# braingeneers/statdepth

Hardware: AMD Instinct MI355X
Metric: curve-pairs/sec (MBD) (higher is better)
Workload: dtype f64

## Files before the change

statdepth_amd/csrc/mbd_rank_bucket32.hip:

```cpp
#include <atomic>

#include "sd_common.h"
#include "rank_bucket.h"

namespace sd {

constexpr int R32_PRIO_LDS = 2;
constexpr int R32_PRIO_VALU = 0;
constexpr int R32_MIN_N = 3072;
constexpr int R32_LNB = 14;
constexpr int R32_NT = 512, R32_NW = 8;
constexpr int R32_LCAP = 64;
constexpr int R32_PAD = 12;
constexpr u32 R32_TB = 1024;
constexpr int R32_TSH = 30;
constexpr double R32_CDIV = 1.0 / 448.0;
constexpr double R32_BETA = 2.0;
constexpr u32 R32_SENT = 0x7FFFFFFFu;

template <int E, int LNB>
struct R32Cfg {
    static constexpr int NT = R32_NT, NW = R32_NW, NB = 1 << LNB;
    static constexpr int QW = NB / 2 / NT / 4;
    static_assert(QW >= 1 && NB / 2 == QW * 4 * NT, "whole quads of histogram words per thread");
    static constexpr int SH = 31 - LNB;
    static constexpr u32 C0 = R32_TB << SH, C1 = ((u32)NB - R32_TB) << SH;
    static constexpr u32 NANIMG = ((u32)NB + 2u) << SH;
    static_assert(LNB == 14, "the first tail octave continues the core's slope for 14 336 core buckets");
    static constexpr size_t HDR = 8 * NW * 8 + NW * 4 + 32 + (size_t)R32_LCAP * 8;
    static_assert(HDR % 16 == 0, "the histogram starts on a 16-byte boundary");
    static __host__ __device__ constexpr int al4(int n) { return (n + 3) & ~3; }
    static __host__ __device__ constexpr int pstride(int n) { return (n + 31) & ~31; }
    static __host__ __device__ constexpr int dummy_pos(int n) { return al4(n) + R32_PAD; }
    static __host__ __device__ constexpr size_t lds_bytes(int n) { return HDR + (size_t)(NB / 2 + 4) * 4 + (size_t)(dummy_pos(n) + 4) * 4; }
};

template <int E, int LNB>
__global__ __launch_bounds__(R32_NT, 4) void rank_bucket32_kernel(const double *__restrict__ Y, i64 n64, i64 row0, i64 rows,
                                                                 u32 *__restrict__ partial, unsigned char *__restrict__ rowflag,
                                                                 u32 *__restrict__ gate, u32 epoch, u64 *__restrict__ out_zero) {
    using C = R32Cfg<E, LNB>;
    constexpr int NT = C::NT, NW = C::NW, NB = C::NB, QW = C::QW, SH = C::SH;
    constexpr u32 C0 = C::C0, C1 = C::C1, NANIMG = C::NANIMG;
    extern __shared__ double Sm[];
    const int n = (int)n64;
    double *red = Sm;
    u32 *wtot = reinterpret_cast<u32 *>(red + 8 * NW);
    u32 *misc = wtot + NW;
    u32 *lkey = misc + 8, *lbe = lkey + R32_LCAP;
    u32 *H = reinterpret_cast<u32 *>(reinterpret_cast<char *>(Sm) + C::HDR);
    u32 *S = H + NB / 2 + 4;
    const unsigned short *H16 = reinterpret_cast<const unsigned short *>(H);
    const int t0 = threadIdx.x;
    const double INF = __builtin_huge_val();
    const double QNAN = __builtin_nan("");
    const int DUMMY = C::dummy_pos(n);
    const uint4 *SENT = reinterpret_cast<const uint4 *>(S + C::al4(n));
    const u32 nm1 = (u32)n - 1u;
    const u32 ranksum = (u32)(((u64)n * (u64)(n - 1)) >> 1);
    int t = t0;

    if (blockIdx.x == 0 && t == 0) gate[2] = 0;
    if (out_zero)
        for (i64 c = (i64)blockIdx.x * NT + t; c < n; c += (i64)gridDim.x * NT) out_zero[c] = 0;
    for (int p = n + t; p < DUMMY + 4; p += NT) S[p] = R32_SENT;
    {
        uint4 *Hq = reinterpret_cast<uint4 *>(H);
#pragma unroll
        for (int i = 0; i < QW; ++i) Hq[i * NT + t] = make_uint4(0, 0, 0, 0);
        if (t < 4) H[NB / 2 + t] = 0;
        if (t < 5) misc[t] = 0;
    }

    double x[E];
    auto load_row = [&](i64 r) {
        const double *rp = Y + (row0 + r) * n + t;
#pragma unroll
        for (int e = 0; e < E; ++e) x[e] = (e < E - 2 || t + e * NT < n) ? rp[e * NT] : QNAN;
    };
    u32 acc[E];
#pragma unroll
    for (int e = 0; e < E; ++e) acc[e] = 0;
    double smp;
    auto sample_issue = [&](i64 r) { smp = Y[(row0 + r) * n + (((((u32)t * 397u) & 511u) * (u32)n) >> 9)]; };
    auto row_range = [&](int parity) {
        double mn = INF, mx = -INF;
#pragma unroll
        for (int e = 0; e < E; ++e) {
            mn = rb_mm<false>(mn, x[e]);
            mx = rb_mm<true>(mx, x[e]);
        }
        mn = rb_wave_allreduce<false>(mn);
        mx = rb_wave_allreduce<true>(mx);
        const float sf = (float)smp;
        const float rmn = rb_row_allreduce_f32<false>(sf == sf ? sf : __builtin_huge_valf());
        const float rmx = rb_row_allreduce_f32<true>(sf == sf ? sf : -__builtin_huge_valf());
        auto rl = [](float v, int l) -> float { return __int_as_float(__builtin_amdgcn_readlane(__float_as_int(v), l)); };
        float imn = fmaxf(fmaxf(rl(rmn, 0), rl(rmn, 16)), fmaxf(rl(rmn, 32), rl(rmn, 48)));
        float imx = fminf(fminf(rl(rmx, 0), rl(rmx, 16)), fminf(rl(rmx, 32), rl(rmx, 48)));
        {
            bool eqs = false;
#define R32_NB(k) eqs = eqs || (__int_as_float(__builtin_amdgcn_mov_dpp(__float_as_int(sf), 0x120 + k, 0xF, 0xF, false)) == sf);
            R32_NB(1) R32_NB(2) R32_NB(3) R32_NB(4) R32_NB(5) R32_NB(6) R32_NB(7)
#undef R32_NB
            if (__ballot(eqs) != 0) { imn = __builtin_huge_valf(); imx = -__builtin_huge_valf(); }
        }
        double *rp = red + parity * 4 * NW;
        if ((t & 63) == 63) {
            double *wp = rp + 4 * (t >> 6);
            wp[0] = mn; wp[1] = mx;
            reinterpret_cast<float *>(wp + 2)[0] = imn;
            reinterpret_cast<float *>(wp + 2)[1] = imx;
        }
    };
    int par = 0;
    u32 rowidx = 0, nbad = 0, expect = 0;
    bool handover = false;
    bool stop = false;
    u32 kb[E];
    i64 r = blockIdx.x;
    for (; r < rows; r += gridDim.x) {
        t = t0;
        asm volatile("" : "+v"(t));
        const int lane = t & 63;
        const int wave = __builtin_amdgcn_readfirstlane(t >> 6);
        if (rowidx && t == 0) misc[3] = __hip_atomic_load(gate + 1, __ATOMIC_RELAXED, __HIP_MEMORY_SCOPE_AGENT);
        __builtin_amdgcn_s_setprio(R32_PRIO_LDS);
        sample_issue(r);
        load_row(r);
        row_range(par);
        double *redp = red + par * 4 * NW;
        par ^= 1;
        __syncthreads();
        if (rowidx) {
            const u32 w = misc[3];
            if ((w >> 8) == (epoch & 0xFFFFFFu) && (w & 0xFFu) >= 8u) { stop = true; break; }
        }
        double lo, hi;
        double mscale, moff, mc;
        u64 mcb;
        u32 mc0, mcw;
        bool go, bad;
        {
            const double2 p = reinterpret_cast<const double2 *>(redp)[2 * (lane & (NW - 1))];
            const float2 pb = reinterpret_cast<const float2 *>(redp + 4 * (lane & (NW - 1)) + 2)[0];
            lo = rb_readlane_f64(rb_row_allreduce<false>(p.x), 0);
            hi = rb_readlane_f64(rb_row_allreduce<true>(p.y), 0);
            const double imn = (double)__int_as_float(__builtin_amdgcn_readfirstlane(__float_as_int(rb_row_allreduce_f32<true>(pb.x))));
            const double imx = (double)__int_as_float(__builtin_amdgcn_readfirstlane(__float_as_int(rb_row_allreduce_f32<false>(pb.y))));
            const bool fin = (hi > lo) && (lo > -INF) && (hi < INF) && ((hi - lo) < INF);
            bad = !fin && (hi >= lo);
            const double si = imx - imn;
            u32 c0 = 256u, c1 = 0x7FFFFE00u;
            if (fin && si > 0.0 && si < INF && (hi - lo) > (1.5 * (1.0 + 2.0 * R32_BETA)) * si) {
                const double lo2 = imn - R32_BETA * si, hi2 = imx + R32_BETA * si;
                lo = lo2 > lo ? lo2 : lo;
                hi = hi2 < hi ? hi2 : hi;
                c0 = C0;
                c1 = C1;
            }
            mc0 = c0;
            mcw = c1 - c0;
            const double wc = hi - lo;
            mscale = ((double)mcw - 64.0) / wc;
            moff = __builtin_fma(-lo, mscale, (double)c0);
            mc = wc * R32_CDIV;
            mcb = (u64)__double_as_longlong(mc);
            go = fin && (wc > 0.0) && (mscale < INF) && (mc > 0.0);
            bad = bad || (fin && !go);
        }
        auto convert4 = [&](const double (&xv)[4], u32 (&q)[4]) {
            bool anyout = false;
#pragma unroll
            for (int i = 0; i < 4; ++i) {
                const double u = __builtin_fma(xv[i], mscale, moff);
                u32 qi;
                asm("v_cvt_u32_f64 %0, %1" : "=v"(qi) : "v"(u));
                q[i] = qi;
                anyout = anyout || (qi - mc0 >= mcw);
            }
            if (__ballot(anyout) != 0) {
#pragma unroll
                for (int i = 0; i < 4; ++i) {
                    const bool outc = q[i] - mc0 >= mcw, low = q[i] < mc0;
                    double d = low ? lo - xv[i] : xv[i] - hi;
                    d = rb_mm<true>(d, 0.0);
                    const u64 tc = ((u64)__double_as_longlong(d + mc) - mcb) >> R32_TSH;
                    const u32 room = low ? mc0 - 1u : 0x7FFFFEFFu - (mc0 + mcw);
                    const u32 tcc = tc < (u64)room ? (u32)tc : room;
                    u32 qt = low ? (mc0 - 1u) - tcc : (mc0 + mcw) + tcc;
                    qt = (xv[i] == xv[i]) ? qt : NANIMG;
                    q[i] = outc ? qt : q[i];
                }
            }
        };
        u32 sl[(E + 3) / 4];
        if (go) {
#pragma unroll
            for (int e = 0; e < (E + 3) / 4; ++e) sl[e] = 0;
#pragma unroll
            for (int e0 = 0; e0 < E; e0 += 8) {
                u32 old[8];
#pragma unroll
                for (int h = 0; h < 8; h += 4) {
                    if (e0 + h < E) {
                        double xv[4];
                        u32 q[4];
#pragma unroll
                        for (int i = 0; i < 4; ++i) xv[i] = e0 + h + i < E ? x[e0 + h + i] : x[e0 + h];
                        convert4(xv, q);
#pragma unroll
                        for (int i = 0; i < 4; ++i)
                            if (e0 + h + i < E) kb[e0 + h + i] = q[i];
                    }
                }
#pragma unroll
                for (int i = 0; i < 8; ++i) {
                    const int e = e0 + i;
                    if (e < E) {
                        const u32 b = kb[e] >> SH;
                        old[i] = atomicAdd(&H[b >> 1], 1u << ((b & 1u) * 16u));
                    }
                }
#pragma unroll
                for (int i = 0; i < 8; ++i) {
                    const int e = e0 + i;
                    if (e < E)
                        sl[e >> 2] |= ((old[i] >> (((kb[e] >> SH) & 1u) * 16u)) & 0xFFu) << (8 * (e & 3));
                }
                asm volatile("" : "+v"(sl[e0 >> 2]));
                if (e0 + 4 < E) asm volatile("" : "+v"(sl[(e0 >> 2) + 1]));
            }
            __syncthreads();
            uint4 *Hq = reinterpret_cast<uint4 *>(H) + wave * (64 * QW);
            uint4 hq[QW];
            u32 runq[QW], inclq[QW], offq[QW], ov = 0, wsum = 0;
#pragma unroll
            for (int i = 0; i < QW; ++i) {
                hq[i] = Hq[i * 64 + lane];
                const u32 s4 = hq[i].x + hq[i].y + hq[i].z + hq[i].w;
                ov |= hq[i].x | hq[i].y | hq[i].z | hq[i].w;
                runq[i] = (s4 & 0xFFFFu) + (s4 >> 16);
                inclq[i] = rb_wave_incl_scan(runq[i]);
                offq[i] = wsum;
                wsum += rb_readlane(inclq[i], 63);
            }
            const bool wover = __ballot((ov & 0xFFC0FFC0u) != 0) != 0;
            const bool wtry = __ballot((ov & 0xFFF0FFF0u) != 0) != 0;
            if (lane == 63) wtot[wave] = wsum | (wover ? 0x80000000u : 0u) | (wtry ? 0x40000000u : 0u);
            __syncthreads();
            const u32 wt = wtot[lane & (NW - 1)];
            const bool crowded = __ballot((wt >> 31) != 0) != 0;
            const bool trypure = __ballot((wt & 0x40000000u) != 0) != 0;
            const u32 wscan = rb_row_incl_scan(wt & 0x3FFFFFFFu);
            const u32 woff = wave ? rb_readlane(wscan, wave - 1) : 0u;
#pragma unroll
            for (int i = 0; i < QW; ++i) {
                u32 base = woff + offq[i] + inclq[i] - runq[i];
                uint4 o;
                o.x = base | ((base + (hq[i].x & 0xFFFFu)) << 16);
                base += (hq[i].x & 0xFFFFu) + (hq[i].x >> 16);
                o.y = base | ((base + (hq[i].y & 0xFFFFu)) << 16);
                base += (hq[i].y & 0xFFFFu) + (hq[i].y >> 16);
                o.z = base | ((base + (hq[i].z & 0xFFFFu)) << 16);
                base += (hq[i].z & 0xFFFFu) + (hq[i].z >> 16);
                o.w = base | ((base + (hq[i].w & 0xFFFFu)) << 16);
                base += (hq[i].w & 0xFFFFu) + (hq[i].w >> 16);
                Hq[i * 64 + lane] = o;
                if (i == QW - 1 && t == NT - 1) H[NB / 2] = base;
            }
            __syncthreads();
            const u32 nv = H[NB / 2];
            bool take = nv == (u32)n;
            u32 bc[E];
            if (take) {
#pragma unroll
                for (int e = 0; e < E; ++e) {
                    const u32 b = kb[e] >> SH, slot = (sl[e >> 2] >> (8 * (e & 3))) & 0xFFu;
                    u32 b1 = b + 1u;
                    asm("" : "+v"(b1));
                    const u32 base = H16[b], end = H16[b1];
                    const bool isk = e < E - 2 || t + e * NT < n;
                    S[isk ? base + slot : (u32)DUMMY] = kb[e];
                    bc[e] = isk ? base | ((end - base) << 14) : (1u << 14);
                }
            }
            __syncthreads();
            bool pure = false;
            if (take && (trypure || crowded)) {
                const u32 tag = rowidx + 1u;
                bool vote = false, same = true;
#pragma unroll
                for (int e = 0; e < E; ++e) {
                    const u32 base = bc[e] & 0x3FFFu, cnt = bc[e] >> 14;
                    if (e < E - 2 || t + e * NT < n) {
                        const u32 first = S[base];
                        same = same && (first == kb[e]);
                        if (cnt >= 16u) vote = vote || (first == kb[e] && S[base + 1] == kb[e]);
                    }
                }
                if (vote) misc[2] = tag;
                if (!same) misc[4] = tag;
                __syncthreads();
                if ((misc[2] == tag && misc[4] != tag) || crowded) {
                    take = false;
                    bool ok = misc[2] == tag && misc[4] != tag;
                    if (ok) {
                        const double *rp = Y + (row0 + r) * n + t;
#pragma unroll
                        for (int pass = 0; pass < 2; ++pass) {
                            bool eq = true;
#pragma unroll
                            for (int e0 = 0; e0 < E; e0 += 4) {
                                int eo = e0 * NT;
                                asm volatile("" : "+v"(eo));
                                const double *rq = rp + eo;
                                u64 w[4];
#pragma unroll
                                for (int i = 0; i < 4; ++i) {
                                    const bool isk = e0 + i < E && (e0 + i < E - 2 || t + (e0 + i) * NT < n);
                                    w[i] = (u64)__double_as_longlong((isk ? rq[i * NT] : 0.0) + 0.0);
                                }
#pragma unroll
                                for (int i = 0; i < 4; ++i) {
                                    if (e0 + i < E && (e0 + i < E - 2 || t + (e0 + i) * NT < n) && (bc[e0 + i] >> 14) >= 2u) {
                                        u32 *sp = S + (bc[e0 + i] & 0x3FFFu);
                                        if (pass == 0) { sp[0] = (u32)(w[i] >> 32); sp[1] = (u32)w[i]; }
                                        else eq = eq && sp[0] == (u32)(w[i] >> 32) && sp[1] == (u32)w[i];
                                    }
                                }
                                __builtin_amdgcn_sched_barrier(0);
                            }
                            if (pass == 1 && !eq) misc[4] = tag;
                            __syncthreads();
                        }
                        ok = misc[4] != tag;
                    }
                    if (ok) {
                        pure = true;
#pragma unroll
                        for (int e = 0; e < E; ++e) {
                            const u32 B = bc[e] & 0x3FFFu, A = (u32)n - B - (bc[e] >> 14);
                            acc[e] += (e < E - 2 || t + e * NT < n) ? (nm1 * (nm1 - 1u) - A * (A - 1u) - B * (B - 1u)) >> 1 : 0u;
                        }
                    }
                }
            }
            __builtin_amdgcn_s_setprio(R32_PRIO_VALU);
            {
                uint4 *Hz = reinterpret_cast<uint4 *>(H) + wave * (64 * QW);
#pragma unroll
                for (int i = 0; i < QW; ++i) Hz[i * 64 + lane] = make_uint4(0, 0, 0, 0);
                if (t < 2) H[NB / 2 + t] = 0;
            }
            if (take) {
                const uint4 *S4 = reinterpret_cast<const uint4 *>(S);
                uint4 y0, y1;
                auto window = [&](int e) {
                    const u32 base = bc[e] & 0x3FFFu, cnt = bc[e] >> 14;
                    const uint4 *p = S4 + (base >> 2);
                    y0 = p[0];
                    y1 = *((cnt + (base & 3u) > 4u) ? p + 1 : SENT);
                };
                u32 sB = 0;
                window(0);
#pragma unroll
                for (int e = 0; e < E; ++e) {
                    const u32 base = bc[e] & 0x3FFFu, cnt = bc[e] >> 14, off = base & 3u;
                    const u32 qe = kb[e];
                    u32 lt = 0;
                    lt = __builtin_amdgcn_alignbit(lt, y0.x - qe, 31);
                    lt = __builtin_amdgcn_alignbit(lt, y0.y - qe, 31);
                    lt = __builtin_amdgcn_alignbit(lt, y0.z - qe, 31);
                    lt = __builtin_amdgcn_alignbit(lt, y0.w - qe, 31);
                    lt = __builtin_amdgcn_alignbit(lt, y1.x - qe, 31);
                    lt = __builtin_amdgcn_alignbit(lt, y1.y - qe, 31);
                    lt = __builtin_amdgcn_alignbit(lt, y1.z - qe, 31);
                    lt = __builtin_amdgcn_alignbit(lt, y1.w - qe, 31);
                    if (e + 1 < E) window(e + 1);
                    u32 less = (u32)__popc(lt);
                    if (cnt + off > 8u) {
                        const uint4 *p = S4 + (base >> 2);
#pragma unroll 1
                        for (u32 kk = 8; kk < cnt + off; kk += 4) {
                            const uint4 y = p[kk >> 2];
                            u32 l4 = 0;
                            l4 = __builtin_amdgcn_alignbit(l4, y.x - qe, 31);
                            l4 = __builtin_amdgcn_alignbit(l4, y.y - qe, 31);
                            l4 = __builtin_amdgcn_alignbit(l4, y.z - qe, 31);
                            l4 = __builtin_amdgcn_alignbit(l4, y.w - qe, 31);
                            less += (u32)__popc(l4);
                        }
                    }
                    const u32 B = base - off + less;
                    kb[e] = B;
                    const bool isk = e < E - 2 || t + e * NT < n;
                    sB += isk ? B : 0u;
                    acc[e] += isk ? __umul24(B, nm1 - B) : 0u;
                    __builtin_amdgcn_sched_barrier(0);
                }
                sB = rb_wave_incl_scan(sB);
                if (lane == 63) atomicAdd(&misc[1], sB);
                __syncthreads();
                {
                    const u32 have_sum = misc[1];
                    expect += ranksum;
                    if (have_sum != expect) {
                        expect = have_sum;
                        const u32 l0 = misc[0];
#pragma unroll
                        for (int e = 0; e < E; ++e)
                            if (e < E - 2 || t + e * NT < n) atomicAdd(&H[kb[e] >> 1], 1u << ((kb[e] & 1u) * 16u));
                        __syncthreads();
#pragma unroll
                        for (int e = 0; e < E; ++e) {
                            if (e < E - 2 || t + e * NT < n) {
                                const u32 B = kb[e], c = H16[B];
                                if (c != 1u) {
                                    acc[e] -= __umul24(B, nm1 - B);
                                    const u32 idx = atomicAdd(&misc[0], 1u);
                                    if (idx < (u32)R32_LCAP) {
                                        lkey[idx] = (rowidx << 14) | (u32)(t + e * NT);
                                        lbe[idx] = B | (c << 16);
                                    }
                                }
                            }
                        }
                        __syncthreads();
                        if (E <= 16 && misc[0] > (u32)R32_LCAP) {
                            const u32 tag = (rowidx + 1u) | 0x40000000u;
                            const double *rp = Y + (row0 + r) * n + t;
#pragma unroll
                            for (int pass = 0; pass < 2; ++pass) {
                                bool eq = true;
#pragma unroll
                                for (int e0 = 0; e0 < E; e0 += 2) {
                                    int eo = e0 * NT;
                                    asm volatile("" : "+v"(eo));
                                    const double *rq = rp + eo;
                                    u64 w[2];
#pragma unroll
                                    for (int i = 0; i < 2; ++i) {
                                        const bool isk = e0 + i < E && (e0 + i < E - 2 || t + (e0 + i) * NT < n);
                                        w[i] = (u64)__double_as_longlong((isk ? rq[i * NT] : 0.0) + 0.0);
                                    }
#pragma unroll
                                    for (int i = 0; i < 2; ++i) {
                                        if (e0 + i < E && (e0 + i < E - 2 || t + (e0 + i) * NT < n) && H16[kb[e0 + i]] >= 2u) {
                                            u32 *sp = S + kb[e0 + i];
                                            if (pass == 0) { sp[0] = (u32)(w[i] >> 32); sp[1] = (u32)w[i]; }
                                            else eq = eq && sp[0] == (u32)(w[i] >> 32) && sp[1] == (u32)w[i];
                                        }
                                    }
                                    __builtin_amdgcn_sched_barrier(0);
                                }
                                if (pass == 1 && !eq) misc[4] = tag;
                                __syncthreads();
                            }
                            if (misc[4] != tag) {
#pragma unroll
                                for (int e = 0; e < E; ++e) {
                                    if (e < E - 2 || t + e * NT < n) {
                                        const u32 B = kb[e], c = H16[B];
                                        if (c != 1u) {
                                            const u32 A = (u32)n - B - c;
                                            acc[e] += (nm1 * (nm1 - 1u) - A * (A - 1u) - B * (B - 1u)) >> 1;
                                        }
                                    }
                                }
                                if (t == 0) misc[0] = l0;
                            }
                            __syncthreads();
                        }
#pragma unroll
                        for (int e = 0; e < E; ++e)
                            if (e < E - 2 || t + e * NT < n) H[kb[e] >> 1] = 0;
                        __syncthreads();
                        if (misc[0] > (u32)R32_LCAP) handover = true;
                    }
                }
            } else {
                bad = !pure;
            }
        }
        if (t == 0) rowflag[r] = bad ? 1 : 0;
        nbad += bad ? 1u : 0u;
        ++rowidx;
        if (handover) break;
        if (bad && rowidx == 1 && t == 0 && blockIdx.x < 16) {
            u32 old = gate[1], assumed;
            do {
                assumed = old;
                const u32 want = ((assumed >> 8) != (epoch & 0xFFFFFFu)) ? (((epoch & 0xFFFFFFu) << 8) | 1u)
                                 : ((assumed & 0xFFu) == 0xFFu ? assumed : assumed + 1u);
                old = atomicCAS(gate + 1, assumed, want);
            } while (old != assumed);
        }
        if (nbad >= 2 && 2 * nbad > rowidx) { stop = true; r += gridDim.x; break; }
    }
    t = t0;
    __syncthreads();
    const u32 L = __builtin_amdgcn_readfirstlane(handover ? 0u : misc[0]);
    if (handover) {
        for (i64 rr = blockIdx.x + (i64)t * gridDim.x; rr < rows; rr += (i64)NT * gridDim.x) rowflag[rr] = 1;
        nbad = 1;
#pragma unroll
        for (int e = 0; e < E; ++e) acc[e] = 0;
    } else if (stop) {
        for (i64 rr = r + (i64)t * gridDim.x; rr < rows; rr += (i64)NT * gridDim.x) rowflag[rr] = 1;
    }
    if (t == 0 && nbad) *gate = epoch;
    u32 key = 0, be = 0;
    double xv = 0.0;
    if ((u32)t < L) {
        key = lkey[t];
        be = lbe[t];
        xv = Y[(row0 + (i64)blockIdx.x + (i64)(key >> 14) * gridDim.x) * n + (key & 0x3FFFu)];
    }
    u32 *P = partial + (size_t)blockIdx.x * C::pstride(n);
#pragma unroll
    for (int e = 0; e < E; ++e)
        if (e < E - 2 || t + e * NT < n) __builtin_nontemporal_store(acc[e], &P[t + e * NT]);
    if (L) {
        asm volatile("s_waitcnt vmcnt(0)" ::: "memory");
        __syncthreads();
        if (t < 64) {
            u32 B = be & 0xFFFFu, A = (u32)n - B - (be >> 16);
            for (u32 j = 0; j < L; ++j) {
                const u32 kj = rb_readlane(key, (int)j), bj = rb_readlane(be, (int)j);
                const double xj = rb_readlane_f64(xv, (int)j);
                if (j != (u32)t && (kj >> 14) == (key >> 14) && (bj & 0xFFFFu) == (be & 0xFFFFu)) {
                    B += (xj < xv) ? 1u : 0u;
                    A += (xj > xv) ? 1u : 0u;
                }
            }
            if ((u32)t < L) atomicAdd(&P[key & 0x3FFFu], (nm1 * (nm1 - 1u) - A * (A - 1u) - B * (B - 1u)) >> 1);
        }
    }
}

bool rank_bucket32_supported(i64 n, i64 rows, int cus) {
    const u64 per = (u64)((rows + cus - 1) / cus) * (u64)n * (u64)n;
    return n > R32_MIN_N && n <= 11264 && rows >= cus && rows <= 4096 && per < ((u64)1 << 32) && xswitch("SD_RB_NO32") == 0;
}

size_t rank_bucket32_extra_bytes(i64 rows) { return align_up((size_t)rows + 64, 256); }

template <int E>
static int launch32_cfg(const double *Y, i64 n, i64 row0, i64 rows, u32 *partial, unsigned char *rowflag, u32 *gate, u32 epoch,
                        u64 *out_zero, int G, hipStream_t s) {
    using C = R32Cfg<E, R32_LNB>;
    auto kf = rank_bucket32_kernel<E, R32_LNB>;
    const size_t lds = C::lds_bytes((int)n);
    if (lds > 81920) return fail(SD_ERR_UNSUPPORTED, "bucket32 kernel: %zu bytes of LDS for n=%lld", lds, (long long)n);
    SD_HIP(hipFuncSetAttribute((const void *)kf, hipFuncAttributeMaxDynamicSharedMemorySize, (int)lds));
    hipLaunchKernelGGL(kf, dim3(G), dim3(R32_NT), lds, s, Y, n, row0, rows, partial, rowflag, gate, epoch, out_zero);
    SD_HIP(hipGetLastError());
    return SD_OK;
}

int launch_rank_bucket32(const double *Y, i64 n, i64 row0, i64 rows, u32 *partial, unsigned char *rowflag, u32 *gate, u32 epoch,
                         u64 *out_zero, int G, hipStream_t s) {
    switch ((int)((n + 1023) / 1024)) {
        case 3: return launch32_cfg<6>(Y, n, row0, rows, partial, rowflag, gate, epoch, out_zero, G, s);
        case 4: return launch32_cfg<8>(Y, n, row0, rows, partial, rowflag, gate, epoch, out_zero, G, s);
        case 5: return launch32_cfg<10>(Y, n, row0, rows, partial, rowflag, gate, epoch, out_zero, G, s);
        case 6: return launch32_cfg<12>(Y, n, row0, rows, partial, rowflag, gate, epoch, out_zero, G, s);
        case 7: return launch32_cfg<14>(Y, n, row0, rows, partial, rowflag, gate, epoch, out_zero, G, s);
        case 8: return launch32_cfg<16>(Y, n, row0, rows, partial, rowflag, gate, epoch, out_zero, G, s);
        case 9: return launch32_cfg<18>(Y, n, row0, rows, partial, rowflag, gate, epoch, out_zero, G, s);
        case 10: return launch32_cfg<20>(Y, n, row0, rows, partial, rowflag, gate, epoch, out_zero, G, s);
        case 11: return launch32_cfg<22>(Y, n, row0, rows, partial, rowflag, gate, epoch, out_zero, G, s);
    }
    return fail(SD_ERR_UNSUPPORTED, "bucket32 kernel covers 3072 < n <= 11264");
}

u32 rank_bucket32_epoch() {
    static std::atomic<u32> counter{0};
    u32 e = ++counter;
    if (e == 0) e = ++counter;
    return e;
}

}
```

Baseline: 2119 billion.

## Refine within-bucket keys with fractional bits and mask comparisons to bucket range

Converts each key into a bucket index plus a refined 31-bit key that includes 14 fractional bits of the scaled value. The bucket index and slot are packed into the existing bc array, which drops the separate sl slot array. The rank comparison now extracts only the bits belonging to the bucket's own range with ubfe rather than counting neighbouring entries and subtracting the offset. This changes the key encoding and the counting logic, and it costs extra fract and convert instructions in the histogram pass.

```diff
diff --git a/statdepth_amd/csrc/mbd_rank_bucket32.hip b/statdepth_amd/csrc/mbd_rank_bucket32.hip
--- a/statdepth_amd/csrc/mbd_rank_bucket32.hip
+++ b/statdepth_amd/csrc/mbd_rank_bucket32.hip
@@ -169,13 +169,16 @@
             go = fin && (wc > 0.0) && (mscale < INF) && (mc > 0.0);
             bad = bad || (fin && !go);
         }
-        auto convert4 = [&](const double (&xv)[4], u32 (&q)[4]) {
+        auto convert4 = [&](const double (&xv)[4], u32 (&q)[4], u32 (&bk)[4]) {
             bool anyout = false;
+            u32 fr[4];
 #pragma unroll
             for (int i = 0; i < 4; ++i) {
                 const double u = __builtin_fma(xv[i], mscale, moff);
                 u32 qi;
                 asm("v_cvt_u32_f64 %0, %1" : "=v"(qi) : "v"(u));
+                const double f = __builtin_amdgcn_fract(u) * 16384.0;
+                asm("v_cvt_u32_f64 %0, %1" : "=v"(fr[i]) : "v"(f));
                 q[i] = qi;
                 anyout = anyout || (qi - mc0 >= mcw);
             }
@@ -191,13 +194,18 @@
                     u32 qt = low ? (mc0 - 1u) - tcc : (mc0 + mcw) + tcc;
                     qt = (xv[i] == xv[i]) ? qt : NANIMG;
                     q[i] = outc ? qt : q[i];
-                }
+                    fr[i] = outc ? 0u : fr[i];
+                }
+            }
+#pragma unroll
+            for (int i = 0; i < 4; ++i) {
+                bk[i] = q[i] >> SH;
+                q[i] = ((q[i] << (31 - SH)) & 0x7FFFFFFFu) | fr[i];
             }
         };
-        u32 sl[(E + 3) / 4];
+        u32 bc[E];
         if (go) {
-#pragma unroll
-            for (int e = 0; e < (E + 3) / 4; ++e) sl[e] = 0;
+
 #pragma unroll
             for (int e0 = 0; e0 < E; e0 += 8) {
                 u32 old[8];
@@ -205,20 +213,20 @@
                 for (int h = 0; h < 8; h += 4) {
                     if (e0 + h < E) {
                         double xv[4];
-                        u32 q[4];
+                        u32 q[4], bk[4];
 #pragma unroll
                         for (int i = 0; i < 4; ++i) xv[i] = e0 + h + i < E ? x[e0 + h + i] : x[e0 + h];
-                        convert4(xv, q);
+                        convert4(xv, q, bk);
 #pragma unroll
                         for (int i = 0; i < 4; ++i)
-                            if (e0 + h + i < E) kb[e0 + h + i] = q[i];
+                            if (e0 + h + i < E) { kb[e0 + h + i] = q[i]; bc[e0 + h + i] = bk[i]; }
                     }
                 }
 #pragma unroll
                 for (int i = 0; i < 8; ++i) {
                     const int e = e0 + i;
                     if (e < E) {
-                        const u32 b = kb[e] >> SH;
+                        const u32 b = bc[e];
                         old[i] = atomicAdd(&H[b >> 1], 1u << ((b & 1u) * 16u));
                     }
                 }
@@ -226,10 +234,11 @@
                 for (int i = 0; i < 8; ++i) {
                     const int e = e0 + i;
                     if (e < E)
-                        sl[e >> 2] |= ((old[i] >> (((kb[e] >> SH) & 1u) * 16u)) & 0xFFu) << (8 * (e & 3));
-                }
-                asm volatile("" : "+v"(sl[e0 >> 2]));
-                if (e0 + 4 < E) asm volatile("" : "+v"(sl[(e0 >> 2) + 1]));
+                        bc[e] |= ((old[i] >> ((bc[e] & 1u) * 16u)) & 0xFFu) << 16;
+                }
+#pragma unroll
+                for (int i = 0; i < 8; ++i)
+                    if (e0 + i < E) asm volatile("" : "+v"(bc[e0 + i]));
             }
             __syncthreads();
             uint4 *Hq = reinterpret_cast<uint4 *>(H) + wave * (64 * QW);
@@ -272,11 +281,10 @@
             __syncthreads();
             const u32 nv = H[NB / 2];
             bool take = nv == (u32)n;
-            u32 bc[E];
             if (take) {
 #pragma unroll
                 for (int e = 0; e < E; ++e) {
-                    const u32 b = kb[e] >> SH, slot = (sl[e >> 2] >> (8 * (e & 3))) & 0xFFu;
+                    const u32 b = bc[e] & 0xFFFFu, slot = bc[e] >> 16;
                     u32 b1 = b + 1u;
                     asm("" : "+v"(b1));
                     const u32 base = H16[b], end = H16[b1];
@@ -369,30 +377,31 @@
                     const u32 base = bc[e] & 0x3FFFu, cnt = bc[e] >> 14, off = base & 3u;
                     const u32 qe = kb[e];
                     u32 lt = 0;
+                    lt = __builtin_amdgcn_alignbit(lt, y1.w - qe, 31);
+                    lt = __builtin_amdgcn_alignbit(lt, y1.z - qe, 31);
+                    lt = __builtin_amdgcn_alignbit(lt, y1.y - qe, 31);
+                    lt = __builtin_amdgcn_alignbit(lt, y1.x - qe, 31);
+                    lt = __builtin_amdgcn_alignbit(lt, y0.w - qe, 31);
+                    lt = __builtin_amdgcn_alignbit(lt, y0.z - qe, 31);
+                    lt = __builtin_amdgcn_alignbit(lt, y0.y - qe, 31);
                     lt = __builtin_amdgcn_alignbit(lt, y0.x - qe, 31);
-                    lt = __builtin_amdgcn_alignbit(lt, y0.y - qe, 31);
-                    lt = __builtin_amdgcn_alignbit(lt, y0.z - qe, 31);
-                    lt = __builtin_amdgcn_alignbit(lt, y0.w - qe, 31);
-                    lt = __builtin_amdgcn_alignbit(lt, y1.x - qe, 31);
-                    lt = __builtin_amdgcn_alignbit(lt, y1.y - qe, 31);
-                    lt = __builtin_amdgcn_alignbit(lt, y1.z - qe, 31);
-                    lt = __builtin_amdgcn_alignbit(lt, y1.w - qe, 31);
                     if (e + 1 < E) window(e + 1);
-                    u32 less = (u32)__popc(lt);
+                    u32 less = (u32)__popc(__builtin_amdgcn_ubfe(lt, off, cnt < 8u ? cnt : 8u));
                     if (cnt + off > 8u) {
                         const uint4 *p = S4 + (base >> 2);
 #pragma unroll 1
                         for (u32 kk = 8; kk < cnt + off; kk += 4) {
                             const uint4 y = p[kk >> 2];
+                            const u32 rest = cnt + off - kk;
                             u32 l4 = 0;
+                            l4 = __builtin_amdgcn_alignbit(l4, y.w - qe, 31);
+                            l4 = __builtin_amdgcn_alignbit(l4, y.z - qe, 31);
+                            l4 = __builtin_amdgcn_alignbit(l4, y.y - qe, 31);
                             l4 = __builtin_amdgcn_alignbit(l4, y.x - qe, 31);
-                            l4 = __builtin_amdgcn_alignbit(l4, y.y - qe, 31);
-                            l4 = __builtin_amdgcn_alignbit(l4, y.z - qe, 31);
-                            l4 = __builtin_amdgcn_alignbit(l4, y.w - qe, 31);
-                            less += (u32)__popc(l4);
+                            less += (u32)__popc(__builtin_amdgcn_ubfe(l4, 0u, rest < 4u ? rest : 4u));
                         }
                     }
-                    const u32 B = base - off + less;
+                    const u32 B = base + less;
                     kb[e] = B;
                     const bool isk = e < E - 2 || t + e * NT < n;
                     sB += isk ? B : 0u;
```

New measurement: 2206 billion (median of 6 runs). 1.04x the previous value.
